# SysCV/sam-pt

Measured on AMD Instinct MI355X. Metric: frames/sec end-to-end (ViT-H + PIPS, 480p, 8 pts, 1 obj) at 1/2/4/8 MI355X, higher is better.
Workload: dtype f16; 1 GPU; SAM vit_h + PIPS, 8 query points, 1 object(s), 24x 480p synthetic frames upscaled to 576x1024, 12 refinement iterations, random-init weights (seed 72); submit=sequential: one blocking SamPt.forward per step, parallelism=sequence-sharded x1, decoder_precision=fp32

## Files before the change

### sam_pt_amd/csrc/attention.hip

```cpp
#include "ops.h"

namespace sampt {

typedef float f32x2 __attribute__((ext_vector_type(2)));

template <typename TQ>
__global__ __launch_bounds__(256) void k_vit_rel_bias(const TQ* __restrict__ qkv, const float* __restrict__ rel_h,
                                                      const float* __restrict__ rel_w, int S, int heads, int hd,
                                                      float* __restrict__ relhT, float* __restrict__ relwT) {
  extern __shared__ float qs[];
  const int qh = blockIdx.x, h = blockIdx.y, b = blockIdx.z;
  const int N = S * S, D = heads * hd, ldq = hd + 1;
  for (int i = threadIdx.x; i < S * hd; i += 256) {
    int t = i / hd, c = i - t * hd;
    qs[t * ldq + c] = (float)qkv[((long)(b * N + qh * S + t)) * 3 * D + h * hd + c];
  }
  __syncthreads();
  const long bh = (long)b * heads + h;
  for (int i = threadIdx.x; i < S * 2 * S; i += 256) {
    int kk = i / S, qw = i - kk * S;
    const float* tab;
    if (kk < S) tab = rel_h + (long)(qh - kk + S - 1) * hd;
    else tab = rel_w + (long)(qw - (kk - S) + S - 1) * hd;
    const float* qv = qs + qw * ldq;
    float a = 0.f;
    for (int c = 0; c < hd; ++c) a += qv[c] * tab[c];
    int q = qh * S + qw;
    if (kk < S) relhT[(bh * S + kk) * N + q] = a;
    else relwT[(bh * S + (kk - S)) * N + q] = a;
  }
}

int vit_rel_bias(const void* qkv, int qkv_f16, const float* rel_h, const float* rel_w, int B, int S, int heads,
                 int hd, float* relh, float* relw, hipStream_t s) {
  dim3 grid(S, heads, B), block(256);
  size_t sh = (size_t)S * (hd + 1) * sizeof(float);
  if (qkv_f16)
    hipLaunchKernelGGL(k_vit_rel_bias<half_t>, grid, block, sh, s, (const half_t*)qkv, rel_h, rel_w, S, heads, hd, relh,
                       relw);
  else
    hipLaunchKernelGGL(k_vit_rel_bias<float>, grid, block, sh, s, (const float*)qkv, rel_h, rel_w, S, heads, hd, relh,
                       relw);
  SAMPT_CHECK_LAUNCH("vit_rel_bias");
  return SAMPT_OK;
}

__global__ __launch_bounds__(256) void k_softmax_rel_rows(float* __restrict__ scores, const float* __restrict__ relhT,
                                                          const float* __restrict__ relwT, int N, int S) {
  __shared__ float red[8];
  const int q = blockIdx.x;
  const long bh = blockIdx.y;
  float* row = scores + (bh * N + q) * N;
  const float* rh = relhT + bh * S * N + q;
  const float* rw = relwT + bh * S * N + q;
  const int tid = threadIdx.x, lane = tid & 63, wave = tid >> 6;
  float m = -INFINITY;
  for (int k = tid; k < N; k += 256) {
    float v = row[k] + rh[(long)(k / S) * N] + rw[(long)(k % S) * N];
    row[k] = v;
    m = fmaxf(m, v);
  }
  m = wave_max(m);
  if (lane == 0) red[wave] = m;
  __syncthreads();
  m = fmaxf(fmaxf(red[0], red[1]), fmaxf(red[2], red[3]));
  float sum = 0.f;
  for (int k = tid; k < N; k += 256) {
    float e = expf(row[k] - m);
    row[k] = e;
    sum += e;
  }
  sum = wave_sum(sum);
  if (lane == 0) red[4 + wave] = sum;
  __syncthreads();
  sum = (red[4] + red[5]) + (red[6] + red[7]);
  for (int k = tid; k < N; k += 256) row[k] = row[k] / sum;
}

int softmax_rel_rows(float* scores, const float* relh, const float* relw, long BH, int Nq, int S, hipStream_t s) {
  if (Nq != S * S) return SAMPT_ERR_ARG;
  hipLaunchKernelGGL(k_softmax_rel_rows, dim3(Nq, (unsigned)BH), dim3(256), 0, s, scores, relh, relw, Nq, S);
  SAMPT_CHECK_LAUNCH("softmax_rel_rows");
  return SAMPT_OK;
}

__device__ half_t g_flash_pad[16] = {(half_t)1.f, (half_t)0.f, (half_t)0.f, (half_t)0.f, (half_t)0.f, (half_t)0.f,
                                     (half_t)0.f, (half_t)0.f, (half_t)0.f, (half_t)0.f, (half_t)0.f, (half_t)0.f,
                                     (half_t)0.f, (half_t)0.f, (half_t)0.f, (half_t)0.f};

template <int HD, int NW, int SG>
__global__ __launch_bounds__(NW * 64, NW == 4 ? 3 : 2) void k_flash_f16(const half_t* __restrict__ qkv, const float* __restrict__ rel_h,
                                                       const float* __restrict__ rel_w, half_t* __restrict__ out, int N,
                                                       int heads, float scale, FlashPad pad, int B, int uh) {
  constexpr int KS = HD / 16;
  constexpr int DT = (HD + 31) / 32;
  constexpr int QT = NW * 32;
  constexpr int NT = NW * 64;
  constexpr bool LROW = DT * 32 > HD;
  constexpr int VP = LROW ? DT * 32 : HD;
  constexpr int RLD = QT + 2;
  constexpr int CPR = HD / 8, CPV = VP / 8;
  constexpr int KSWZ = CPR == 8 ? 7 : (CPR == 4 ? 3 : (CPR == 10 ? 1 : 0)), KSH = CPR == 4 ? 2 : (CPR == 10 ? 3 : 1);
  constexpr int KB = 64 * HD * 2, VB = 64 * VP * 2, RELB = SG * RLD * 2;
  constexpr int BUFB = KB + VB > RELB ? KB + VB : ((RELB + 1023) / 1024) * 1024;
  __shared__ __attribute__((aligned(1024))) char tile_s[BUFB];
  __shared__ half_t relh_s[SG][RLD];
  half_t(*Ks)[64][HD] = (half_t(*)[64][HD])tile_s;
  half_t(*Vs)[64][VP] = (half_t(*)[64][VP])(tile_s + KB);
  half_t(*relw_s)[RLD] = (half_t(*)[RLD])tile_s;
  constexpr int NKI = (CPR + NW - 1) / NW, NVI = (CPV + NW - 1) / NW;
  __shared__ unsigned dma_tab[NKI + NVI][NT];

  const int tid = threadIdx.x, lane = tid & 63, wave = __builtin_amdgcn_readfirstlane(tid >> 6);
  const int li = lane & 31, hi = lane >> 5;
  int bx, h, b;
  flash_wg_decode(blockIdx.x, (N + QT - 1) / QT, heads, B, uh, bx, h, b);
  const int D = heads * HD;
  const long tok0 = (long)b * N;
  const int qblk = bx * QT;
  const int ql = wave * 32 + li;
  const int q = qblk + ql;
  const bool wave_live = qblk + wave * 32 < N;
  constexpr int RPT = SG >= 64 ? 1 : 64 / SG, KTV = SG >= 64 ? 64 : RPT * SG;
  constexpr float LOG2E = 1.4426950408889634f;
  const float c2 = scale * LOG2E;
  const int pw = pad.bias_row ? b % pad.nwin : 0;
  const int pwy = pw / max(pad.nwx, 1), py0 = pwy * SG, px0 = (pw - pwy * max(pad.nwx, 1)) * SG;
  auto is_pad = [&](int t) {
    const int iy = t / SG, ix = t - iy * SG;
    return pad.bias_row != nullptr && (py0 + iy >= pad.gh || px0 + ix >= pad.gw);
  };
  {
    int n = 0;
    for (int i = wave; i < CPR; i += NW, ++n) {
      const int e = i * 64 + lane, slot = e / CPR, c = e - slot * CPR;
      const int sc = min(slot, KTV - 1), siy = sc / SG, six = sc - siy * SG;
      const unsigned off = (unsigned)((c ^ ((slot >> KSH) & KSWZ)) * 16);
      dma_tab[n][tid] = (unsigned)sc | (unsigned)siy << 8 | (pad.bias_row != nullptr && px0 + six >= pad.gw ? 1u << 12 : 0u) | off << 16;
    }
    n = NKI;
    for (int i = wave; i < CPV; i += NW, ++n) {
      const int e = i * 64 + lane, slot = e / CPV, c = e - slot * CPV;
      const int sc = min(slot, KTV - 1), siy = sc / SG, six = sc - siy * SG;
      const int cs = HD == 64 ? c ^ (((slot >> 1) & 1) << 2) : c;
      const unsigned off = (unsigned)(c < CPR ? cs * 16 : (c - CPR) * 16);
      dma_tab[n][tid] = (unsigned)sc | (unsigned)siy << 8 | (pad.bias_row != nullptr && px0 + six >= pad.gw ? 1u << 12 : 0u) |
                        (c < CPR ? 0u : 1u << 13) | off << 16;
    }
  }
  auto dma_tile = [&](int kt0, int kh0, int buf) {
    const half_t* kbase = qkv + tok0 * 3 * D + D + h * HD;
    const unsigned stride = 3u * (unsigned)D * 2u;
    const char* kb = (const char*)kbase;
    const char* vb = (const char*)(kbase + D);
    const char* pk = (const char*)(pad.bias_row ? pad.bias_row + D + h * HD : kbase);
    const char* pv = (const char*)(pad.bias_row ? pad.bias_row + 2 * D + h * HD : kbase);
    int n = 0;
    for (int i = wave; i < CPR; i += NW, ++n) {
      const unsigned t = dma_tab[n][tid];
      const unsigned krow = min((unsigned)kt0 + (t & 255u), (unsigned)(N - 1));
      const int gr = kh0 + (int)(t >> 8 & 15u);
      const bool pd = pad.bias_row != nullptr && ((t & 0x1000u) != 0 || gr >= SG || py0 + gr >= pad.gh);
      const char* src = pd ? pk + (t >> 16) : kb + (__umul24(krow, stride) + (t >> 16));
      __builtin_amdgcn_global_load_lds((const __attribute__((address_space(1))) void*)src,
                                       (__attribute__((address_space(3))) void*)((char*)&Ks[buf][0][0] + i * 1024), 16, 0, 0);
    }
    n = NKI;
    for (int i = wave; i < CPV; i += NW, ++n) {
      const unsigned t = dma_tab[n][tid];
      const unsigned vrow = min((unsigned)kt0 + (t & 255u), (unsigned)(N - 1));
      const int gr = kh0 + (int)(t >> 8 & 15u);
      const bool pd = pad.bias_row != nullptr && ((t & 0x1000u) != 0 || gr >= SG || py0 + gr >= pad.gh);
      const char* src = pd ? pv + (t >> 16) : vb + (__umul24(vrow, stride) + (t >> 16));
      if (LROW && (t & 0x2000u)) src = (const char*)g_flash_pad + (t >> 16);
      __builtin_amdgcn_global_load_lds((const __attribute__((address_space(1))) void*)src,
                                       (__attribute__((address_space(3))) void*)((char*)&Vs[buf][0][0] + i * 1024), 16, 0, 0);
    }
  };

  for (int i = tid; i < SG * RLD; i += NT) {
    (&relh_s[0][0])[i] = (half_t)0.f;
    (&relw_s[0][0])[i] = (half_t)0.f;
  }
  h8 qf[KS];
#pragma unroll
  for (int ks = 0; ks < KS; ++ks) {
    if (q < N && !is_pad(q)) qf[ks] = *(const h8*)(qkv + (tok0 + q) * 3 * D + h * HD + ks * 16 + hi * 8);
    else qf[ks] = (h8){0, 0, 0, 0, 0, 0, 0, 0};
  }
  __syncthreads();
  {
    constexpr int NR = 2 * SG - 1, NTIL = (NR + 31) / 32;
    const int qh = q / SG, qw = q - qh * SG;
#pragma unroll
    for (int tb = 0; tb < 2; ++tb) {
      const float* tab = tb == 0 ? rel_h : rel_w;
      const int qpos = tb == 0 ? qh : qw;
#pragma unroll
      for (int t = 0; t < NTIL; ++t) {
        f32x16 g;
#pragma unroll
        for (int r = 0; r < 16; ++r) g[r] = 0.f;
        const int row = 32 * t + li;
#pragma unroll
        for (int ks = 0; ks < KS; ++ks) {
          h8 tf = (h8){0, 0, 0, 0, 0, 0, 0, 0};
          if (pad.rel_ops) {
            tf = *(const h8*)(pad.rel_ops + ((((long)tb * NTIL + t) * KS + ks) * 64 + lane) * 8);
          } else if (row < NR) {
            const float4* tp = (const float4*)(tab + (long)row * HD + ks * 16 + hi * 8);
            float4 t0 = tp[0], t1 = tp[1];
            tf = (h8){(half_t)t0.x, (half_t)t0.y, (half_t)t0.z, (half_t)t0.w,
                      (half_t)t1.x, (half_t)t1.y, (half_t)t1.z, (half_t)t1.w};
          }
          g = __builtin_amdgcn_mfma_f32_32x32x16_f16(tf, qf[ks], g, 0, 0, 0);
        }
        if (q < N) {
#pragma unroll
          for (int r = 0; r < 16; ++r) {
            const int rho = 32 * t + (r & 3) + 8 * (r >> 2) + 4 * hi;
            const int kx = qpos - rho + SG - 1;
            if (kx >= 0 && kx < SG) {
              if (tb == 0) relh_s[kx][ql] = (half_t)g[r];
              else relw_s[kx][ql] = (half_t)g[r];
            }
          }
        }
      }
    }
  }

  f32x16 o[DT];
#pragma unroll
  for (int dt = 0; dt < DT; ++dt)
#pragma unroll
    for (int r = 0; r < 16; ++r) o[dt][r] = 0.f;
  float m_run = -INFINITY, l_run = 0.f;

  __syncthreads();
  float relw2[32];
#pragma unroll
  for (int kt = 0; kt < 2; ++kt)
#pragma unroll
    for (int r = 0; r < 16; ++r) {
      const int j = kt * 32 + (r & 3) + 8 * (r >> 2) + 4 * hi;
      const int kw = SG >= 64 ? j : j % SG;
      relw2[kt * 16 + r] = j < KTV ? LOG2E * (float)relw_s[kw][ql] : -INFINITY;
    }

  int vl[DT];
  {
    const int s16 = li & 15, r4 = s16 >> 2, cc = s16 & 3, g16 = li >> 4;
#pragma unroll
    for (int dt = 0; dt < DT; ++dt)
      vl[dt] = (4 * hi + r4) * VP * 2 + ((dt * 64 + g16 * 32 + cc * 8) ^ (HD == 64 ? ((r4 >> 1) & 1) << 6 : 0));
  }
  __syncthreads();
  dma_tile(0, 0, 0);
  asm volatile("s_waitcnt vmcnt(0)" ::: "memory");
  __syncthreads();
  for (int kt0 = 0, kh0 = 0, it = 0; kt0 < N; kt0 += KTV, kh0 += RPT, ++it) {
    constexpr int buf = 0;
    if (wave_live) {
    const bool half1 = RPT == 1 || kh0 + 32 / SG < SG;

    f32x16 st[2];
#pragma unroll
    for (int kt = 0; kt < 2; ++kt) {
#pragma unroll
      for (int r = 0; r < 16; ++r) st[kt][r] = 0.f;
      if (kt == 1 && !half1) continue;
#pragma unroll
      for (int ks = 0; ks < KS; ++ks) {
        const int krow = kt * 32 + li;
        h8 kf = *(const h8*)&Ks[buf][krow][((ks * 2 + hi) ^ ((krow >> KSH) & KSWZ)) * 8];
        st[kt] = __builtin_amdgcn_mfma_f32_32x32x16_f16(kf, qf[ks], st[kt], 0, 0, 0);
      }
    }
    float rh[RPT];
#pragma unroll
    for (int jr = 0; jr < RPT; ++jr) rh[jr] = kh0 + jr < SG ? LOG2E * (float)relh_s[kh0 + jr][ql] : -INFINITY;
    float mloc = -INFINITY;
    f32x2 sv2[2][8];
    const f32x2 c2v = (f32x2){c2, c2};
#pragma unroll
    for (int kt = 0; kt < 2; ++kt) {
#pragma unroll
      for (int rp = 0; rp < 8; ++rp) {
        f32x2 x = (f32x2){st[kt][2 * rp], st[kt][2 * rp + 1]};
        x = x * c2v + (f32x2){relw2[kt * 16 + 2 * rp], relw2[kt * 16 + 2 * rp + 1]};
        if (RPT > 1) {
          f32x2 bb;
#pragma unroll
          for (int e = 0; e < 2; ++e) {
            const int r = 2 * rp + e;
            const int j0 = kt * 32 + (r & 3) + 8 * (r >> 2);
            const int ja = min(j0 / SG, RPT - 1), jb = min((j0 + 4) / SG, RPT - 1);
            bb[e] = ja == jb ? rh[ja] : (hi ? rh[jb] : rh[ja]);
          }
          x = x + bb;
        }
        sv2[kt][rp] = x;
        mloc = fmaxf(mloc, fmaxf(x[0], x[1]));
      }
    }
    if (RPT == 1) mloc += rh[0];
    mloc = fmaxf(mloc, __shfl_xor(mloc, 32, 64));
    const float m_new = fmaxf(m_run, mloc);
    const float msub = RPT == 1 ? m_new - rh[0] : m_new;
    const f32x2 mv = (f32x2){msub, msub};
    float lsum = 0.f;
    h8 pb[4];
#pragma unroll
    for (int kt = 0; kt < 2; ++kt) {
      if (kt == 1 && !half1) continue;
#pragma unroll
      for (int r = 0; r < 16; r += 2) {
        const f32x2 e2 = sv2[kt][r >> 1] - mv;
        const float p0 = __builtin_amdgcn_exp2f(e2[0]), p1 = __builtin_amdgcn_exp2f(e2[1]);
        if (!LROW) lsum += p0 + p1;
        f32x2 pp = (f32x2){p0, p1};
        h2 ph = __builtin_convertvector(pp, h2);
        pb[kt * 2 + (r >> 3)][r & 7] = ph[0];
        pb[kt * 2 + (r >> 3)][(r & 7) + 1] = ph[1];
      }
    }
    if (!LROW) lsum += __shfl_xor(lsum, 32, 64);
    if (__any(m_new > m_run)) {
      const float alpha = __builtin_amdgcn_exp2f(m_run - m_new);
      l_run *= alpha;
#pragma unroll
      for (int dt = 0; dt < DT; ++dt)
#pragma unroll
        for (int r = 0; r < 16; ++r) o[dt][r] *= alpha;
      m_run = m_new;
    }
    l_run += lsum;
#pragma unroll
    for (int t = 0; t < 4; ++t) {
      if (t >= 2 && !half1) continue;
#pragma unroll
      for (int dt = 0; dt < DT; ++dt) {
        typedef short s4 __attribute__((ext_vector_type(4)));
        typedef __attribute__((address_space(3))) s4 lds_s4;
        const __attribute__((address_space(3))) char* vb =
            (const __attribute__((address_space(3))) char*)&Vs[buf][0][0] + vl[dt] + 16 * t * VP * 2;
        const s4 v0 = __builtin_amdgcn_ds_read_tr16_b64_v4i16((lds_s4*)vb);
        const s4 v1 = __builtin_amdgcn_ds_read_tr16_b64_v4i16((lds_s4*)(vb + 8 * VP * 2));
        const h8 vf = __builtin_bit_cast(h8, __builtin_shufflevector(v0, v1, 0, 1, 2, 3, 4, 5, 6, 7));
        o[dt] = __builtin_amdgcn_mfma_f32_32x32x16_f16(vf, pb[t], o[dt], 0, 0, 0);
      }
    }
    }
    if (kt0 + KTV < N) {
      __syncthreads();
      dma_tile(kt0 + KTV, kh0 + RPT, 0);
    }
    asm volatile("s_waitcnt vmcnt(0)" ::: "memory");
    __syncthreads();
  }

  if (LROW) {
    constexpr int LR = HD % 32, RL = (LR % 4) + 4 * (LR / 8), HL = (LR / 4) % 2;
    l_run = __shfl(o[DT - 1][RL], li | (HL << 5), 64);
  }
  if (q < N) {
    const float inv = 1.0f / l_run;
    half_t* op = out + (tok0 + q) * D + h * HD;
#pragma unroll
    for (int dt = 0; dt < DT; ++dt) {
#pragma unroll
      for (int g = 0; g < 4; ++g) {
        int d0 = dt * 32 + 8 * g + 4 * hi;
        if (d0 < HD) {
          h4 v = (h4){(half_t)(o[dt][4 * g] * inv), (half_t)(o[dt][4 * g + 1] * inv), (half_t)(o[dt][4 * g + 2] * inv),
                      (half_t)(o[dt][4 * g + 3] * inv)};
          *(h4*)(op + d0) = v;
        }
      }
    }
  }
}

int vit_flash_attention_f16(const half_t* qkv, const float* relh, const float* relw, half_t* out, int B, int S,
                            int heads, int hd, hipStream_t s, FlashPad pad) {
  if (pad.bias_row && (pad.nwx <= 0 || pad.nwin <= 0 || B % pad.nwin)) return SAMPT_ERR_ARG;
  const int N = S * S;
  const float scale = 1.0f / sqrtf((float)hd);
#define FL(HDv, NWv, SGv)                                                                                     \
  hipLaunchKernelGGL((k_flash_f16<HDv, NWv, SGv>), dim3(cdiv(N, NWv * 32) * heads * B), dim3(NWv * 64), 0, s, qkv, relh, relw, \
                     out, N, heads, scale, pad, B, SGv < 64 ? heads : 0)
  if (S == 64 && hd == 80) FL(80, 4, 64);
  else if (S == 64 && hd == 64) FL(64, 4, 64);
  else if (S == 14 && hd == 80) FL(80, 4, 14);
  else if (S == 14 && hd == 64) FL(64, 4, 14);
  else if (S == 16 && hd == 32) FL(32, 4, 16);
  else if (S == 6 && hd == 32) FL(32, 2, 6);
  else return SAMPT_ERR_UNSUPPORTED;
#undef FL
  SAMPT_CHECK_LAUNCH("vit_flash_attention_f16");
  return SAMPT_OK;
}

}
```

### sam_pt_amd/csrc/attention_x3.hip

```cpp
#include "ops.h"

namespace sampt {

typedef float f32x2 __attribute__((ext_vector_type(2)));

__device__ half_t g_flash_pad_x3[16] = {(half_t)1.f, (half_t)0.f, (half_t)0.f, (half_t)0.f, (half_t)0.f, (half_t)0.f,
                                        (half_t)0.f, (half_t)0.f, (half_t)0.f, (half_t)0.f, (half_t)0.f, (half_t)0.f,
                                        (half_t)0.f, (half_t)0.f, (half_t)0.f, (half_t)0.f};

template <int HD, int NW, int SG>
struct FlashX3Geom {
  static constexpr int DT = (HD + 31) / 32;
  static constexpr bool LROW = DT * 32 > HD;
  static constexpr int VP = LROW ? DT * 32 : HD;
  static constexpr int QT = NW * 32, RLD = QT + 2;
  static constexpr int K_PLANE = 64 * HD * 2, V_PLANE = 64 * VP * 2;
  static constexpr int BUF = 2 * K_PLANE + 2 * V_PLANE;
  static constexpr int REL = SG * RLD * 4;
  static constexpr int TILES = BUF > REL ? BUF : REL;
  static constexpr int LDS = TILES + REL;
};

template <int HD, int NW, int SG>
__global__ __launch_bounds__(NW * 64, 2) void k_flash_x3(const half_t* __restrict__ qkv, const float* __restrict__ rel_h,
                                                         const float* __restrict__ rel_w, half_t* __restrict__ out, int N,
                                                         int heads, float scale, FlashPad pad, int B, int uh) {
  typedef FlashX3Geom<HD, NW, SG> G;
  constexpr int KS = HD / 16;
  constexpr int DT = G::DT;
  constexpr int QT = G::QT;
  constexpr int NT = NW * 64;
  constexpr bool LROW = G::LROW;
  constexpr int VP = G::VP;
  constexpr int RLD = G::RLD;
  constexpr int CPR = HD / 8, CPV = VP / 8;
  constexpr int KSWZ = CPR == 8 ? 7 : (CPR == 4 ? 3 : (CPR == 10 ? 1 : 0)), KSH = CPR == 4 ? 2 : (CPR == 10 ? 3 : 1);
  extern __shared__ __attribute__((aligned(1024))) char smem[];
  auto Kp = [&](int b, int p) -> char* { return smem + b * G::BUF + p * G::K_PLANE; };
  auto Vp = [&](int b, int p) -> char* { return smem + b * G::BUF + 2 * G::K_PLANE + p * G::V_PLANE; };
  float* relh_s = (float*)(smem + G::TILES);
  float* relw_s = (float*)smem;

  const int tid = threadIdx.x, lane = tid & 63, wave = __builtin_amdgcn_readfirstlane(tid >> 6);
  const int li = lane & 31, hi = lane >> 5;
  int bx, h, b;
  flash_wg_decode(blockIdx.x, (N + QT - 1) / QT, heads, B, uh, bx, h, b);
  const int D = heads * HD;
  const long ldq = 6L * D;
  const long tok0 = (long)b * N;
  const int qblk = bx * QT;
  const int ql = wave * 32 + li;
  const int q = qblk + ql;
  const bool wave_live = qblk + wave * 32 < N;
  constexpr int RPT = SG >= 64 ? 1 : 64 / SG, KTV = SG >= 64 ? 64 : RPT * SG;
  constexpr float LOG2E = 1.4426950408889634f;
  const float c2 = scale * LOG2E;

  auto xcol = [](int c) -> int { return ((c >> 5) << 6) + (c & 31); };
  const int pw = pad.bias_row ? b % pad.nwin : 0;
  const int pwy = pw / max(pad.nwx, 1), py0 = pwy * SG, px0 = (pw - pwy * max(pad.nwx, 1)) * SG;
  auto is_pad = [&](int t) {
    const int iy = t / SG, ix = t - iy * SG;
    return pad.bias_row != nullptr && (py0 + iy >= pad.gh || px0 + ix >= pad.gw);
  };
  auto dma_tile = [&](int kt0, int buf) {
    const half_t* rbase = qkv + tok0 * ldq;
#pragma unroll
    for (int pl = 0; pl < 2; ++pl) {
      for (int i = wave; i < CPR; i += NW) {
        const int e = i * 64 + lane, slot = e / CPR, c = e - slot * CPR;
        const int krow = min(kt0 + min(slot, KTV - 1), N - 1);
        const half_t* rowp = is_pad(krow) ? pad.bias_row : rbase + (long)krow * ldq;
        const half_t* src = rowp + xcol(D + h * HD + ((c ^ ((slot >> KSH) & KSWZ)) * 8)) + pl * 32;
        __builtin_amdgcn_global_load_lds((const __attribute__((address_space(1))) void*)src,
                                         (__attribute__((address_space(3))) void*)(Kp(buf, pl) + i * 1024), 16, 0, 0);
      }
      for (int i = wave; i < CPV; i += NW) {
        const int e = i * 64 + lane, slot = e / CPV, c = e - slot * CPV;
        const int vrow = min(kt0 + min(slot, KTV - 1), N - 1);
        const int cs = HD == 64 ? c ^ (((slot >> 1) & 1) << 2) : c;
        const half_t* rowp = is_pad(vrow) ? pad.bias_row : rbase + (long)vrow * ldq;
        const half_t* src = c < CPR ? rowp + xcol(2 * D + h * HD + cs * 8) + pl * 32
                                    : g_flash_pad_x3 + (pl == 0 ? (c - CPR) * 8 : 8);
        __builtin_amdgcn_global_load_lds((const __attribute__((address_space(1))) void*)src,
                                         (__attribute__((address_space(3))) void*)(Vp(buf, pl) + i * 1024), 16, 0, 0);
      }
    }
  };

  for (int i = tid; i < SG * RLD; i += NT) relh_s[i] = 0.f, relw_s[i] = 0.f;
  h8 qh[KS], qlo[KS];
#pragma unroll
  for (int ks = 0; ks < KS; ++ks) {
    if (q < N && !is_pad(q)) {
      const half_t* qp = qkv + (tok0 + q) * ldq + xcol(h * HD + ks * 16 + hi * 8);
      qh[ks] = *(const h8*)qp;
      qlo[ks] = *(const h8*)(qp + 32);
    } else {
      qh[ks] = qlo[ks] = (h8){0, 0, 0, 0, 0, 0, 0, 0};
    }
  }
  __syncthreads();
  {
    constexpr int NR = 2 * SG - 1, NTIL = (NR + 31) / 32;
    const int qhh = q / SG, qw = q - qhh * SG;
#pragma unroll
    for (int tb = 0; tb < 2; ++tb) {
      const float* tab = tb == 0 ? rel_h : rel_w;
      const int qpos = tb == 0 ? qhh : qw;
      float* dst = tb == 0 ? relh_s : relw_s;
#pragma unroll
      for (int t = 0; t < NTIL; ++t) {
        f32x16 g;
#pragma unroll
        for (int r = 0; r < 16; ++r) g[r] = 0.f;
        const int row = 32 * t + li;
#pragma unroll
        for (int ks = 0; ks < KS; ++ks) {
          h8 th = (h8){0, 0, 0, 0, 0, 0, 0, 0}, tl = th;
          if (row < NR) {
            const float4* tp = (const float4*)(tab + (long)row * HD + ks * 16 + hi * 8);
            const float4 t0 = tp[0], t1 = tp[1];
            const float tv[8] = {t0.x, t0.y, t0.z, t0.w, t1.x, t1.y, t1.z, t1.w};
#pragma unroll
            for (int e = 0; e < 8; ++e) {
              half_t a, bb;
              split_f16(tv[e], a, bb);
              th[e] = a, tl[e] = bb;
            }
          }
          g = __builtin_amdgcn_mfma_f32_32x32x16_f16(tl, qh[ks], g, 0, 0, 0);
          g = __builtin_amdgcn_mfma_f32_32x32x16_f16(th, qlo[ks], g, 0, 0, 0);
          g = __builtin_amdgcn_mfma_f32_32x32x16_f16(th, qh[ks], g, 0, 0, 0);
        }
        if (q < N) {
#pragma unroll
          for (int r = 0; r < 16; ++r) {
            const int rho = 32 * t + (r & 3) + 8 * (r >> 2) + 4 * hi;
            const int kx = qpos - rho + SG - 1;
            if (kx >= 0 && kx < SG) dst[kx * RLD + ql] = g[r];
          }
        }
      }
    }
  }

  f32x16 o[DT];
#pragma unroll
  for (int dt = 0; dt < DT; ++dt)
#pragma unroll
    for (int r = 0; r < 16; ++r) o[dt][r] = 0.f;
  float m_run = -INFINITY, l_run = 0.f;

  __syncthreads();
  float relw2[32];
#pragma unroll
  for (int kt = 0; kt < 2; ++kt)
#pragma unroll
    for (int r = 0; r < 16; ++r) {
      const int j = kt * 32 + (r & 3) + 8 * (r >> 2) + 4 * hi;
      const int kw = SG >= 64 ? j : j % SG;
      relw2[kt * 16 + r] = j < KTV ? LOG2E * relw_s[kw * RLD + ql] : -INFINITY;
    }

  int vl[DT];
  {
    const int s16 = li & 15, r4 = s16 >> 2, cc = s16 & 3, g16 = li >> 4;
#pragma unroll
    for (int dt = 0; dt < DT; ++dt)
      vl[dt] = (4 * hi + r4) * VP * 2 + ((dt * 64 + g16 * 32 + cc * 8) ^ (HD == 64 ? ((r4 >> 1) & 1) << 6 : 0));
  }
  __syncthreads();
  dma_tile(0, 0);
  asm volatile("s_waitcnt vmcnt(0)" ::: "memory");
  __syncthreads();
  for (int kt0 = 0, kh0 = 0, it = 0; kt0 < N; kt0 += KTV, kh0 += RPT, ++it) {
    constexpr int buf = 0;
    if (wave_live) {
    const bool half1 = RPT == 1 || HD == 64 || kh0 + 32 / SG < SG;

    f32x16 st[2];
#pragma unroll
    for (int kt = 0; kt < 2; ++kt) {
#pragma unroll
      for (int r = 0; r < 16; ++r) st[kt][r] = 0.f;
      if (kt == 1 && !half1) continue;
#pragma unroll
      for (int ks = 0; ks < KS; ++ks) {
        const int krow = kt * 32 + li;
        const int off = (krow * HD + ((ks * 2 + hi) ^ ((krow >> KSH) & KSWZ)) * 8) * 2;
        const h8 kfh = *(const h8*)(Kp(buf, 0) + off);
        const h8 kfl = *(const h8*)(Kp(buf, 1) + off);
        st[kt] = __builtin_amdgcn_mfma_f32_32x32x16_f16(kfl, qh[ks], st[kt], 0, 0, 0);
        st[kt] = __builtin_amdgcn_mfma_f32_32x32x16_f16(kfh, qlo[ks], st[kt], 0, 0, 0);
        st[kt] = __builtin_amdgcn_mfma_f32_32x32x16_f16(kfh, qh[ks], st[kt], 0, 0, 0);
      }
    }
    float rh[RPT];
#pragma unroll
    for (int jr = 0; jr < RPT; ++jr) rh[jr] = kh0 + jr < SG ? LOG2E * relh_s[(kh0 + jr) * RLD + ql] : -INFINITY;
    float mloc = -INFINITY;
    f32x2 sv2[2][8];
    const f32x2 c2v = (f32x2){c2, c2};
#pragma unroll
    for (int kt = 0; kt < 2; ++kt) {
#pragma unroll
      for (int rp = 0; rp < 8; ++rp) {
        f32x2 x = (f32x2){st[kt][2 * rp], st[kt][2 * rp + 1]};
        x = x * c2v + (f32x2){relw2[kt * 16 + 2 * rp], relw2[kt * 16 + 2 * rp + 1]};
        if (RPT > 1) {
          f32x2 bb;
#pragma unroll
          for (int e = 0; e < 2; ++e) {
            const int r = 2 * rp + e;
            const int j0 = kt * 32 + (r & 3) + 8 * (r >> 2);
            const int ja = min(j0 / SG, RPT - 1), jb = min((j0 + 4) / SG, RPT - 1);
            bb[e] = ja == jb ? rh[ja] : (hi ? rh[jb] : rh[ja]);
          }
          x = x + bb;
        }
        sv2[kt][rp] = x;
        mloc = fmaxf(mloc, fmaxf(x[0], x[1]));
      }
    }
    if (RPT == 1) mloc += rh[0];
    mloc = fmaxf(mloc, __shfl_xor(mloc, 32, 64));
    const float m_new = fmaxf(m_run, mloc);
    constexpr float PSH = 15.f;
    const float msub = (RPT == 1 ? m_new - rh[0] : m_new) - PSH;
    const f32x2 mv = (f32x2){msub, msub};
    float lsum = 0.f;
    h8 pbh[4], pbl[4];
#pragma unroll
    for (int kt = 0; kt < 2; ++kt) {
      if (kt == 1 && !half1) continue;
#pragma unroll
      for (int r = 0; r < 16; r += 2) {
        const f32x2 e2 = sv2[kt][r >> 1] - mv;
        const float p0 = __builtin_amdgcn_exp2f(e2[0]), p1 = __builtin_amdgcn_exp2f(e2[1]);
        if (!LROW) lsum += p0 + p1;
        const f32x2 pp = (f32x2){p0, p1};
        const h2 ph = __builtin_convertvector(pp, h2);
        const f32x2 pr = pp - __builtin_convertvector(ph, f32x2);
        const h2 pl = __builtin_convertvector(pr, h2);
        pbh[kt * 2 + (r >> 3)][r & 7] = ph[0];
        pbh[kt * 2 + (r >> 3)][(r & 7) + 1] = ph[1];
        pbl[kt * 2 + (r >> 3)][r & 7] = pl[0];
        pbl[kt * 2 + (r >> 3)][(r & 7) + 1] = pl[1];
      }
    }
    if (!LROW) lsum += __shfl_xor(lsum, 32, 64);
    if (__any(m_new > m_run)) {
      const float alpha = __builtin_amdgcn_exp2f(m_run - m_new);
      l_run *= alpha;
#pragma unroll
      for (int dt = 0; dt < DT; ++dt)
#pragma unroll
        for (int r = 0; r < 16; ++r) o[dt][r] *= alpha;
      m_run = m_new;
    }
    l_run += lsum;
#pragma unroll
    for (int t = 0; t < 4; ++t) {
      if (t >= 2 && !half1) continue;
#pragma unroll
      for (int dt = 0; dt < DT; ++dt) {
        typedef short s4 __attribute__((ext_vector_type(4)));
        typedef __attribute__((address_space(3))) s4 lds_s4;
        h8 vf[2];
#pragma unroll
        for (int pl = 0; pl < 2; ++pl) {
          const __attribute__((address_space(3))) char* vb =
              (const __attribute__((address_space(3))) char*)Vp(buf, pl) + vl[dt] + 16 * t * VP * 2;
          const s4 v0 = __builtin_amdgcn_ds_read_tr16_b64_v4i16((lds_s4*)vb);
          const s4 v1 = __builtin_amdgcn_ds_read_tr16_b64_v4i16((lds_s4*)(vb + 8 * VP * 2));
          vf[pl] = __builtin_bit_cast(h8, __builtin_shufflevector(v0, v1, 0, 1, 2, 3, 4, 5, 6, 7));
        }
        o[dt] = __builtin_amdgcn_mfma_f32_32x32x16_f16(vf[1], pbh[t], o[dt], 0, 0, 0);
        o[dt] = __builtin_amdgcn_mfma_f32_32x32x16_f16(vf[0], pbl[t], o[dt], 0, 0, 0);
        o[dt] = __builtin_amdgcn_mfma_f32_32x32x16_f16(vf[0], pbh[t], o[dt], 0, 0, 0);
      }
    }
    }
    if (kt0 + KTV < N) {
      __syncthreads();
      dma_tile(kt0 + KTV, 0);
    }
    asm volatile("s_waitcnt vmcnt(0)" ::: "memory");
    __syncthreads();
  }

  if (LROW) {
    constexpr int LR = HD % 32, RL = (LR % 4) + 4 * (LR / 8), HL = (LR / 4) % 2;
    l_run = __shfl(o[DT - 1][RL], li | (HL << 5), 64);
  }
  if (q < N) {
    const float inv = 1.0f / l_run;
    half_t* op = out + (tok0 + q) * 2 * D;
#pragma unroll
    for (int dt = 0; dt < DT; ++dt) {
#pragma unroll
      for (int g = 0; g < 4; ++g) {
        const int d0 = dt * 32 + 8 * g + 4 * hi;
        if (d0 < HD) {
          h4 vh, vlo;
#pragma unroll
          for (int e = 0; e < 4; ++e) {
            half_t a, bb;
            split_f16(o[dt][4 * g + e] * inv, a, bb);
            vh[e] = a, vlo[e] = bb;
          }
          half_t* p = op + xcol(h * HD + d0);
          *(h4*)p = vh;
          *(h4*)(p + 32) = vlo;
        }
      }
    }
  }
}

int vit_flash_attention_x3(const half_t* qkv, const float* relh, const float* relw, half_t* out, int B, int S, int heads,
                           int hd, hipStream_t s, FlashPad pad) {
  if (pad.bias_row && (pad.nwx <= 0 || pad.nwin <= 0 || B % pad.nwin)) return SAMPT_ERR_ARG;
  const int N = S * S;
  const float scale = 1.0f / sqrtf((float)hd);
  if ((heads * hd) % 32) return SAMPT_ERR_UNSUPPORTED;
#define FLX(HDv, NWv, SGv)                                                                                              \
  do {                                                                                                                  \
    typedef FlashX3Geom<HDv, NWv, SGv> G;                                                                               \
    static bool raised = false;                                                                                         \
    auto kern = k_flash_x3<HDv, NWv, SGv>;                                                                              \
    if (!raised) {                                                                                                      \
      if (hipFuncSetAttribute((const void*)kern, hipFuncAttributeMaxDynamicSharedMemorySize, G::LDS) != hipSuccess)     \
        return SAMPT_ERR_HIP;                                                                                           \
      raised = true;                                                                                                    \
    }                                                                                                                   \
    hipLaunchKernelGGL(kern, dim3(cdiv(N, NWv * 32) * heads * B), dim3(NWv * 64), G::LDS, s, qkv, relh, relw, out, N,   \
                       heads, scale, pad, B, SGv < 64 ? heads : 0);                   \
  } while (0)
  if (S == 64 && hd == 80) FLX(80, 4, 64);
  else if (S == 64 && hd == 64) FLX(64, 4, 64);
  else if (S == 14 && hd == 80) FLX(80, 4, 14);
  else if (S == 14 && hd == 64) FLX(64, 4, 14);
  else if (S == 16 && hd == 32) FLX(32, 4, 16);
  else if (S == 6 && hd == 32) FLX(32, 2, 6);
  else return SAMPT_ERR_UNSUPPORTED;
#undef FLX
  SAMPT_CHECK_LAUNCH("vit_flash_attention_x3");
  return SAMPT_OK;
}

}
```

### sam_pt_amd/csrc/common.h

```cpp
#pragma once
#include <hip/hip_runtime.h>
#include <stdint.h>

#include "gelu_poly.h"

#define SAMPT_OK 0
#define SAMPT_ERR_ARG (-1)
#define SAMPT_ERR_HIP (-2)
#define SAMPT_ERR_UNSUPPORTED (-3)
#define SAMPT_ERR_WORKSPACE (-4)

typedef _Float16 half_t;
typedef float f32x4 __attribute__((ext_vector_type(4)));
typedef float f32x16 __attribute__((ext_vector_type(16)));
typedef _Float16 h8 __attribute__((ext_vector_type(8)));
typedef _Float16 h4 __attribute__((ext_vector_type(4)));
typedef _Float16 h2 __attribute__((ext_vector_type(2)));

namespace sampt {

void set_error(const char* where, hipError_t e);
const char* last_error();

#define SAMPT_CHECK_LAUNCH(name)                                   \
  do {                                                             \
    hipError_t _e = hipGetLastError();                             \
    if (_e != hipSuccess) { sampt::set_error(name, _e); return SAMPT_ERR_HIP; } \
  } while (0)

#define SAMPT_TRY(expr)                          \
  do {                                           \
    int _rc = (expr);                            \
    if (_rc != SAMPT_OK) return _rc;             \
  } while (0)

enum Act { ACT_NONE = 0, ACT_RELU = 1, ACT_GELU = 2, ACT_GELU_TANH = 3 };

__device__ __forceinline__ float gelu_erf(float x) {
  return 0.5f * x * (1.0f + erff(x * 0.70710678118654752440f));
}

__device__ __forceinline__ float gelu_tanh(float x) {
  const float inner = 0.79788456080286535588f * (x + 0.044715f * x * x * x);
  return 0.5f * x * (1.0f + tanhf(inner));
}

__device__ __forceinline__ float apply_act(float x, int act) {
  if (act == ACT_RELU) return x > 0.f ? x : 0.f;
  if (act == ACT_GELU) return gelu_erf(x);
  if (act == ACT_GELU_TANH) return gelu_tanh(x);
  return x;
}

__device__ __forceinline__ float wave_sum(float v) {
#pragma unroll
  for (int o = 32; o > 0; o >>= 1) v += __shfl_xor(v, o, 64);
  return v;
}
__device__ __forceinline__ float wave_max(float v) {
#pragma unroll
  for (int o = 32; o > 0; o >>= 1) v = fmaxf(v, __shfl_xor(v, o, 64));
  return v;
}
__device__ __forceinline__ double wave_sum_d(double v) {
#pragma unroll
  for (int o = 32; o > 0; o >>= 1) v += __shfl_xor(v, o, 64);
  return v;
}

__device__ __forceinline__ void split_f16(float v, half_t& hi, half_t& lo) {
  hi = (half_t)__builtin_amdgcn_fmed3f(v, -65504.f, 65504.f);
  lo = (half_t)(v - (float)hi);
}
__device__ __forceinline__ long x3_col(int c) { return ((long)(c >> 5) << 6) + (c & 31); }

__device__ __forceinline__ void flash_wg_decode(int L, int nx, int heads, int B, int uh, int& x, int& h, int& b) {
  if (uh <= 0) {
    x = L % nx;
    const int t = L / nx;
    h = t % heads, b = t / heads;
    return;
  }
  const int hg = heads / uh, units = B * hg, pu = uh * nx, full = units & ~7;
  int unit, r;
  if (L < full * pu) {
    const int j = L >> 3;
    unit = (j / pu) * 8 + (L & 7), r = j % pu;
  } else {
    const int lt = L - full * pu;
    unit = full + lt / pu, r = lt % pu;
  }
  b = unit / hg;
  h = (unit % hg) * uh + r / nx;
  x = r % nx;
}

typedef float f32x2_g __attribute__((ext_vector_type(2)));
__device__ __forceinline__ float gelu_fast(float x) {
  const float z = fabsf(x) * 0.70710678118654752440f;
  const float t = __builtin_amdgcn_rcpf(fmaf(0.3275911f, z, 1.0f));
  float pl = fmaf(1.061405429f, t, -1.453152027f);
  pl = fmaf(pl, t, 1.421413741f);
  pl = fmaf(pl, t, -0.284496736f);
  pl = fmaf(pl, t, 0.254829592f);
  const float e = pl * t * __builtin_amdgcn_exp2f(z * z * -1.44269504088896340736f);
  const float phi = x < 0.f ? 0.5f * e : 1.0f - 0.5f * e;
  return x * phi;
}

__device__ __forceinline__ f32x2_g gelu_poly2(f32x2_g x) {
  constexpr float cf[GELU_POLY_DEG + 1] = GELU_POLY_COEFS;
  const f32x2_g xc = {__builtin_amdgcn_fmed3f(x[0], -GELU_POLY_C, GELU_POLY_C), __builtin_amdgcn_fmed3f(x[1], -GELU_POLY_C, GELU_POLY_C)};
  const float k = 2.0f / (GELU_POLY_C * GELU_POLY_C);
  const f32x2_g t = xc * xc * (f32x2_g){k, k} - (f32x2_g){1.f, 1.f};
  f32x2_g pl = {cf[GELU_POLY_DEG], cf[GELU_POLY_DEG]};
#pragma unroll
  for (int i = GELU_POLY_DEG - 1; i >= 0; --i) pl = pl * t + (f32x2_g){cf[i], cf[i]};
  return x * (xc * pl + (f32x2_g){0.5f, 0.5f});
}

__device__ __forceinline__ float gelu_half_gemm(float v, int out_f16) {
  return out_f16 == 1 ? gelu_poly2((f32x2_g){v, v})[0] : gelu_fast(v);
}

static inline int cdiv(long a, long b) { return (int)((a + b - 1) / b); }

struct GemmP {
  const void* A = nullptr;
  const void* W = nullptr;
  const void* W_lo = nullptr;
  const void* A_lo = nullptr;
  const float* bias = nullptr;
  const float* res = nullptr;
  void* C = nullptr;
  const int* rowmap = nullptr;
  const int* a_rowmap = nullptr;
  int M = 0, N = 0, K = 0;
  int lda = 0, ldw = 0, ldc = 0, ldr = 0;
  int nb1 = 1, nb2 = 1;
  long sA1 = 0, sA2 = 0, sW1 = 0, sW2 = 0, sC1 = 0, sC2 = 0;
  long sRowmap1 = 0;
  int res_mod = 0;
  int shuf_g = 0, shuf_n = 0;
  int act = ACT_NONE;
  int out_f16 = 0;
  int x3 = 0;
  int w_kn = 0;
  float alpha = 1.0f;
  int xcd_swizzle = 0;
  int p8_wgs = 0;
  int p8_stagger = 0;
  int force_generic = 0;
  int splitk = 1;
  float* splitk_ws = nullptr;
  size_t splitk_ws_floats = 0;
  int conv = 0;
  int cH = 0, cW = 0, cC = 0, KH = 0, KW = 0, cstride = 1, cpad = 0, OH = 0, OW = 0;
  int cpadw = -1;
  double* in_part = nullptr;
  int epi = 0;
  const float* epi_a = nullptr;
  const float* epi_b = nullptr;
  float epi_eps = 0.f;
  int epi_ld = 0;
};

extern int g_p8_sched;
extern int g_p8_stagger;
extern int g_p8_trim;
extern int g_thin_min_wgs;
int gemm_f32(const GemmP& p, hipStream_t s);
int gemm_f16(const GemmP& p, hipStream_t s);
int gemm_f32_plan_splitk(const GemmP& p);
#define F16X3_WSHIFT 8
int conv_f16x3(const GemmP& p, hipStream_t s);
extern int g_conv_halo;
extern int g_halo_dbg;
extern int g_conv_in_stats;
bool conv3x3_halo_eligible(const GemmP& p);
extern int g_gemm_x3_wres;
extern int g_gemm_x3_epi;
bool gemm_x3_wres_eligible(const GemmP& p);
int gemm_x3_wres(const GemmP& p, hipStream_t s);
bool gemm_x3_wres_ln_eligible(const GemmP& p);
int conv3x3_halo_x3(const GemmP& p, hipStream_t s);
int conv3x3_halo_tiles(const GemmP& p);

}
```

Baseline: 121.8 frames/s.

## Launch flash attention workgroups only for real query rows in padded windows

Adds a host-side plan that classifies windows into full, right-edge, bottom-edge and corner classes and counts only the query tiles holding real tokens. The kernels decode this compacted grid and remap compact query indices back to window positions, skipping workgroups and rows that were pure padding. This cuts wasted attention work in padded edge windows. In exchange it adds index arithmetic and a stricter nwin % nwx argument check, and padded output rows are no longer written.

```diff
diff --git a/sam_pt_amd/csrc/attention.hip b/sam_pt_amd/csrc/attention.hip
--- a/sam_pt_amd/csrc/attention.hip
+++ b/sam_pt_amd/csrc/attention.hip
@@ -91,7 +91,7 @@
 template <int HD, int NW, int SG>
 __global__ __launch_bounds__(NW * 64, NW == 4 ? 3 : 2) void k_flash_f16(const half_t* __restrict__ qkv, const float* __restrict__ rel_h,
                                                        const float* __restrict__ rel_w, half_t* __restrict__ out, int N,
-                                                       int heads, float scale, FlashPad pad, int B, int uh) {
+                                                       int heads, float scale, FlashPad pad, int B, int uh, FlashRealQ rq) {
   constexpr int KS = HD / 16;
   constexpr int DT = (HD + 31) / 32;
   constexpr int QT = NW * 32;
@@ -114,22 +114,27 @@
   const int tid = threadIdx.x, lane = tid & 63, wave = __builtin_amdgcn_readfirstlane(tid >> 6);
   const int li = lane & 31, hi = lane >> 5;
   int bx, h, b;
-  flash_wg_decode(blockIdx.x, (N + QT - 1) / QT, heads, B, uh, bx, h, b);
+  int nrx = SG, nq = N;
+  if (pad.bias_row) {
+    int nry;
+    flash_realq_decode(blockIdx.x, rq, SG, heads, B / pad.nwin, pad.nwx, pad.nwin, bx, h, b, nry, nrx);
+    nq = nry * nrx;
+  } else {
+    flash_wg_decode(blockIdx.x, (N + QT - 1) / QT, heads, B, uh, bx, h, b);
+  }
   const int D = heads * HD;
   const long tok0 = (long)b * N;
   const int qblk = bx * QT;
   const int ql = wave * 32 + li;
-  const int q = qblk + ql;
-  const bool wave_live = qblk + wave * 32 < N;
+  const int qc = qblk + ql;
+  const bool q_live = qc < nq;
+  const int q = nrx == SG ? qc : qc + (qc / nrx) * (SG - nrx);
+  const bool wave_live = qblk + wave * 32 < nq;
   constexpr int RPT = SG >= 64 ? 1 : 64 / SG, KTV = SG >= 64 ? 64 : RPT * SG;
   constexpr float LOG2E = 1.4426950408889634f;
   const float c2 = scale * LOG2E;
   const int pw = pad.bias_row ? b % pad.nwin : 0;
   const int pwy = pw / max(pad.nwx, 1), py0 = pwy * SG, px0 = (pw - pwy * max(pad.nwx, 1)) * SG;
-  auto is_pad = [&](int t) {
-    const int iy = t / SG, ix = t - iy * SG;
-    return pad.bias_row != nullptr && (py0 + iy >= pad.gh || px0 + ix >= pad.gw);
-  };
   {
     int n = 0;
     for (int i = wave; i < CPR; i += NW, ++n) {
@@ -185,7 +190,7 @@
   h8 qf[KS];
 #pragma unroll
   for (int ks = 0; ks < KS; ++ks) {
-    if (q < N && !is_pad(q)) qf[ks] = *(const h8*)(qkv + (tok0 + q) * 3 * D + h * HD + ks * 16 + hi * 8);
+    if (q_live) qf[ks] = *(const h8*)(qkv + (tok0 + q) * 3 * D + h * HD + ks * 16 + hi * 8);
     else qf[ks] = (h8){0, 0, 0, 0, 0, 0, 0, 0};
   }
   __syncthreads();
@@ -215,7 +220,7 @@
           }
           g = __builtin_amdgcn_mfma_f32_32x32x16_f16(tf, qf[ks], g, 0, 0, 0);
         }
-        if (q < N) {
+        if (q_live) {
 #pragma unroll
           for (int r = 0; r < 16; ++r) {
             const int rho = 32 * t + (r & 3) + 8 * (r >> 2) + 4 * hi;
@@ -364,7 +369,7 @@
     constexpr int LR = HD % 32, RL = (LR % 4) + 4 * (LR / 8), HL = (LR / 4) % 2;
     l_run = __shfl(o[DT - 1][RL], li | (HL << 5), 64);
   }
-  if (q < N) {
+  if (q_live) {
     const float inv = 1.0f / l_run;
     half_t* op = out + (tok0 + q) * D + h * HD;
 #pragma unroll
@@ -384,12 +389,21 @@
 
 int vit_flash_attention_f16(const half_t* qkv, const float* relh, const float* relw, half_t* out, int B, int S,
                             int heads, int hd, hipStream_t s, FlashPad pad) {
-  if (pad.bias_row && (pad.nwx <= 0 || pad.nwin <= 0 || B % pad.nwin)) return SAMPT_ERR_ARG;
+  if (pad.bias_row && (pad.nwx <= 0 || pad.nwin <= 0 || pad.nwin % pad.nwx || B % pad.nwin)) return SAMPT_ERR_ARG;
   const int N = S * S;
   const float scale = 1.0f / sqrtf((float)hd);
+  if (B <= 0) return SAMPT_ERR_ARG;
+  auto plan = [&](int QT) {
+    return pad.bias_row ? flash_realq_plan(S, pad.nwx, pad.nwin / pad.nwx, pad.gh, pad.gw, B / pad.nwin, heads, QT) : FlashRealQ();
+  };
 #define FL(HDv, NWv, SGv)                                                                                     \
-  hipLaunchKernelGGL((k_flash_f16<HDv, NWv, SGv>), dim3(cdiv(N, NWv * 32) * heads * B), dim3(NWv * 64), 0, s, qkv, relh, relw, \
-                     out, N, heads, scale, pad, B, SGv < 64 ? heads : 0)
+  do {                                                                                                        \
+    const FlashRealQ rq = plan(NWv * 32);                                                                     \
+    const int nwg = pad.bias_row ? rq.end[3] : cdiv(N, NWv * 32) * heads * B;                                 \
+    if (nwg > 0)                                                \
+      hipLaunchKernelGGL((k_flash_f16<HDv, NWv, SGv>), dim3(nwg), dim3(NWv * 64), 0, s, qkv, relh, relw, out, N, heads, scale, \
+                         pad, B, SGv < 64 ? heads : 0, rq);                                                   \
+  } while (0)
   if (S == 64 && hd == 80) FL(80, 4, 64);
   else if (S == 64 && hd == 64) FL(64, 4, 64);
   else if (S == 14 && hd == 80) FL(80, 4, 14);
diff --git a/sam_pt_amd/csrc/attention_x3.hip b/sam_pt_amd/csrc/attention_x3.hip
--- a/sam_pt_amd/csrc/attention_x3.hip
+++ b/sam_pt_amd/csrc/attention_x3.hip
@@ -24,7 +24,7 @@
 template <int HD, int NW, int SG>
 __global__ __launch_bounds__(NW * 64, 2) void k_flash_x3(const half_t* __restrict__ qkv, const float* __restrict__ rel_h,
                                                          const float* __restrict__ rel_w, half_t* __restrict__ out, int N,
-                                                         int heads, float scale, FlashPad pad, int B, int uh) {
+                                                         int heads, float scale, FlashPad pad, int B, int uh, FlashRealQ rq) {
   typedef FlashX3Geom<HD, NW, SG> G;
   constexpr int KS = HD / 16;
   constexpr int DT = G::DT;
@@ -44,14 +44,23 @@
   const int tid = threadIdx.x, lane = tid & 63, wave = __builtin_amdgcn_readfirstlane(tid >> 6);
   const int li = lane & 31, hi = lane >> 5;
   int bx, h, b;
-  flash_wg_decode(blockIdx.x, (N + QT - 1) / QT, heads, B, uh, bx, h, b);
+  int nrx = SG, nq = N;
+  if (pad.bias_row) {
+    int nry;
+    flash_realq_decode(blockIdx.x, rq, SG, heads, B / pad.nwin, pad.nwx, pad.nwin, bx, h, b, nry, nrx);
+    nq = nry * nrx;
+  } else {
+    flash_wg_decode(blockIdx.x, (N + QT - 1) / QT, heads, B, uh, bx, h, b);
+  }
   const int D = heads * HD;
   const long ldq = 6L * D;
   const long tok0 = (long)b * N;
   const int qblk = bx * QT;
   const int ql = wave * 32 + li;
-  const int q = qblk + ql;
-  const bool wave_live = qblk + wave * 32 < N;
+  const int qc = qblk + ql;
+  const bool q_live = qc < nq;
+  const int q = nrx == SG ? qc : qc + (qc / nrx) * (SG - nrx);
+  const bool wave_live = qblk + wave * 32 < nq;
   constexpr int RPT = SG >= 64 ? 1 : 64 / SG, KTV = SG >= 64 ? 64 : RPT * SG;
   constexpr float LOG2E = 1.4426950408889634f;
   const float c2 = scale * LOG2E;
@@ -92,7 +101,7 @@
   h8 qh[KS], qlo[KS];
 #pragma unroll
   for (int ks = 0; ks < KS; ++ks) {
-    if (q < N && !is_pad(q)) {
+    if (q_live) {
       const half_t* qp = qkv + (tok0 + q) * ldq + xcol(h * HD + ks * 16 + hi * 8);
       qh[ks] = *(const h8*)qp;
       qlo[ks] = *(const h8*)(qp + 32);
@@ -133,7 +142,7 @@
           g = __builtin_amdgcn_mfma_f32_32x32x16_f16(th, qlo[ks], g, 0, 0, 0);
           g = __builtin_amdgcn_mfma_f32_32x32x16_f16(th, qh[ks], g, 0, 0, 0);
         }
-        if (q < N) {
+        if (q_live) {
 #pragma unroll
           for (int r = 0; r < 16; ++r) {
             const int rho = 32 * t + (r & 3) + 8 * (r >> 2) + 4 * hi;
@@ -294,7 +303,7 @@
     constexpr int LR = HD % 32, RL = (LR % 4) + 4 * (LR / 8), HL = (LR / 4) % 2;
     l_run = __shfl(o[DT - 1][RL], li | (HL << 5), 64);
   }
-  if (q < N) {
+  if (q_live) {
     const float inv = 1.0f / l_run;
     half_t* op = out + (tok0 + q) * 2 * D;
 #pragma unroll
@@ -321,10 +330,11 @@
 
 int vit_flash_attention_x3(const half_t* qkv, const float* relh, const float* relw, half_t* out, int B, int S, int heads,
                            int hd, hipStream_t s, FlashPad pad) {
-  if (pad.bias_row && (pad.nwx <= 0 || pad.nwin <= 0 || B % pad.nwin)) return SAMPT_ERR_ARG;
+  if (pad.bias_row && (pad.nwx <= 0 || pad.nwin <= 0 || pad.nwin % pad.nwx || B % pad.nwin)) return SAMPT_ERR_ARG;
   const int N = S * S;
   const float scale = 1.0f / sqrtf((float)hd);
   if ((heads * hd) % 32) return SAMPT_ERR_UNSUPPORTED;
+  if (B <= 0) return SAMPT_ERR_ARG;
 #define FLX(HDv, NWv, SGv)                                                                                              \
   do {                                                                                                                  \
     typedef FlashX3Geom<HDv, NWv, SGv> G;                                                                               \
@@ -335,8 +345,13 @@
         return SAMPT_ERR_HIP;                                                                                           \
       raised = true;                                                                                                    \
     }                                                                                                                   \
-    hipLaunchKernelGGL(kern, dim3(cdiv(N, NWv * 32) * heads * B), dim3(NWv * 64), G::LDS, s, qkv, relh, relw, out, N,   \
-                       heads, scale, pad, B, SGv < 64 ? heads : 0);                   \
+                                       \
+    const FlashRealQ rq = pad.bias_row ? flash_realq_plan(S, pad.nwx, pad.nwin / pad.nwx, pad.gh, pad.gw, B / pad.nwin, \
+                                                          heads, NWv * 32) : FlashRealQ();                              \
+    const int nwg = pad.bias_row ? rq.end[3] : cdiv(N, NWv * 32) * heads * B;                                           \
+    if (nwg > 0)                                                                                                        \
+      hipLaunchKernelGGL(kern, dim3(nwg), dim3(NWv * 64), G::LDS, s, qkv, relh, relw, out, N, heads, scale, pad, B,     \
+                         SGv < 64 ? heads : 0, rq);                                                                     \
   } while (0)
   if (S == 64 && hd == 80) FLX(80, 4, 64);
   else if (S == 64 && hd == 64) FLX(64, 4, 64);
diff --git a/sam_pt_amd/csrc/common.h b/sam_pt_amd/csrc/common.h
--- a/sam_pt_amd/csrc/common.h
+++ b/sam_pt_amd/csrc/common.h
@@ -93,6 +93,44 @@
   b = unit / hg;
   h = (unit % hg) * uh + r / nx;
   x = r % nx;
+}
+
+struct FlashRealQ {
+  int cfx = 0, cfy = 0;
+  int nrx_e = 0, nry_e = 0;
+  int nxb[4] = {0, 0, 0, 0};
+  int end[4] = {0, 0, 0, 0};
+};
+__host__ __device__ __forceinline__ int flash_realq_cw(const FlashRealQ& r, int k) { return (k & 1) ? (r.nrx_e > 0) : r.cfx; }
+__host__ __device__ __forceinline__ int flash_realq_ch(const FlashRealQ& r, int k) { return (k & 2) ? (r.nry_e > 0) : r.cfy; }
+
+static inline FlashRealQ flash_realq_plan(int S, int nwx, int nwy, int gh, int gw, int frames, int heads, int QT) {
+  FlashRealQ r;
+  gh = gh < 0 ? 0 : gh, gw = gw < 0 ? 0 : gw;
+  r.cfx = gw / S < nwx ? gw / S : nwx, r.cfy = gh / S < nwy ? gh / S : nwy;
+  r.nrx_e = r.cfx < nwx ? gw - r.cfx * S : 0, r.nry_e = r.cfy < nwy ? gh - r.cfy * S : 0;
+  int e = 0;
+  for (int k = 0; k < 4; ++k) {
+    const int nq = ((k & 2) ? r.nry_e : S) * ((k & 1) ? r.nrx_e : S);
+    r.nxb[k] = (nq + QT - 1) / QT;
+    e += frames * flash_realq_cw(r, k) * flash_realq_ch(r, k) * heads * r.nxb[k];
+    r.end[k] = e;
+  }
+  return r;
+}
+
+__device__ __forceinline__ void flash_realq_decode(int L, const FlashRealQ& r, int S, int heads, int frames, int nwx, int nwin,
+                                                   int& x, int& h, int& b, int& nry, int& nrx) {
+  const int k = (L >= r.end[0]) + (L >= r.end[1]) + (L >= r.end[2]);
+  const int start = k == 0 ? 0 : (k == 1 ? r.end[0] : (k == 2 ? r.end[1] : r.end[2]));
+  const int nx = k == 0 ? r.nxb[0] : (k == 1 ? r.nxb[1] : (k == 2 ? r.nxb[2] : r.nxb[3]));
+  const int cw = flash_realq_cw(r, k), wc = cw * flash_realq_ch(r, k);
+  int bl;
+  flash_wg_decode(L - start, nx, heads, frames * wc, heads, x, h, bl);
+  const int f = bl / wc, wi = bl - f * wc, wr = wi / cw;
+  const int wy = ((k & 2) ? r.cfy : 0) + wr, wx = ((k & 1) ? r.cfx : 0) + (wi - wr * cw);
+  b = f * nwin + wy * nwx + wx;
+  nry = (k & 2) ? r.nry_e : S, nrx = (k & 1) ? r.nrx_e : S;
 }
 
 typedef float f32x2_g __attribute__((ext_vector_type(2)));
```

After: 122.8 frames/s (median of 6 runs). About the same (+0.8%).
